# IDEA-CCNL/Fengshenbang-LM

Measured on NVIDIA H100. Metric: tokens_per_sec, higher is better.
Workload: dtype bf16

## Files before the change

fengshen-lm_b200/csrc/attention_bwd.cu:

```cuda
#include "host_common.h"
#include "ptx.cuh"

namespace fsb {

int make_attn_tmap(CUtensorMap* tm, const void* base, int64_t row_stride, int64_t width, int64_t seq, int64_t batch,
                   int box_rows);

constexpr int AB_THREADS = 384;
constexpr int AB_BM = 128;
constexpr int AB_BN = 64;
constexpr int AB_NDIAG = AB_BM + AB_BN - 1;
constexpr int AB_DSTRIDE = 192;

struct AttBwdParams {
  const float* lse;
  const float* delta;
  const uint8_t* kv_mask;
  const float* rel_bias;
  float* dbias_part;
  __nv_bfloat16 *dq, *dk, *dv;
  int64_t dq_row_stride, dk_row_stride, dv_row_stride, dq_head_stride, dk_head_stride, dv_head_stride;
  int q_head_stride, k_head_stride, v_head_stride, do_head_stride;
  int seq_q, seq_kv, nheads, batch, causal;
  float scale, scale_log2;
};

template <int D>
__global__ void __launch_bounds__(256) attn_delta_kernel(const __nv_bfloat16* __restrict__ o,
                                                         const __nv_bfloat16* __restrict__ dout, float* __restrict__ delta,
                                                         int64_t o_row_stride, int64_t o_head_stride,
                                                         int64_t do_row_stride, int64_t do_head_stride, int batch, int seq,
                                                         int nheads) {
  constexpr int G = D / 8;
  const int64_t gid = (blockIdx.x * int64_t(blockDim.x) + threadIdx.x) / G;
  const int gl = threadIdx.x % G;
  const int64_t total = int64_t(batch) * seq * nheads;
  float s = 0.f;
  int64_t bs = 0; int h = 0;
  if (gid < total) {
    h = int(gid % nheads);
    bs = gid / nheads;
    float a[8], b[8];
    unpack8(*reinterpret_cast<const uint4*>(o + bs * o_row_stride + h * o_head_stride + gl * 8), a);
    unpack8(*reinterpret_cast<const uint4*>(dout + bs * do_row_stride + h * do_head_stride + gl * 8), b);
#pragma unroll
    for (int j = 0; j < 8; ++j) s += a[j] * b[j];
  }
#pragma unroll
  for (int off = G / 2; off > 0; off >>= 1) s += __shfl_xor_sync(0xffffffffu, s, off);
  if (gid < total && gl == 0) {
    const int64_t b = bs / seq, sq = bs % seq;
    delta[(b * nheads + h) * seq + sq] = s;
  }
}

template <int D, bool kDS>
struct AttBwdSmem {
  static constexpr int BIG_BYTES = AB_BM * D * 2;
  static constexpr int SML_BYTES = AB_BN * D * 2;
  static constexpr int STAGES = 3;
  static constexpr int OFF_BIG0 = 0;
  static constexpr int OFF_BIG1 = OFF_BIG0 + BIG_BYTES;
  static constexpr int OFF_SML0 = OFF_BIG1 + BIG_BYTES;
  static constexpr int OFF_SML1 = OFF_SML0 + STAGES * SML_BYTES;
  static constexpr int OFF_DS = OFF_SML1 + STAGES * SML_BYTES;
  static constexpr int OFF_BAR = OFF_DS + (kDS ? (AB_BM * (AB_BN + 1) * 4 + 15) / 16 * 16 : 0);
  static constexpr int NBAR = 1 + 2 * STAGES;
  static constexpr int TOTAL = OFF_BAR + NBAR * 8 + 1024;
  static_assert(TOTAL <= 232448, "exceeds the 227 KB of shared memory a block can opt into on sm_90");
};

template <int D>
__device__ __forceinline__ void wgmma_rs_acc(float (&o)[D / 2], const uint32_t (&a)[4], uint64_t db) {
  if constexpr (D == 128) wgmma_rs_n128<1>(o, a, db, 1u);
  else wgmma_rs_n64<1>(o, a, db, 1u);
}
__device__ __forceinline__ uint32_t kslice(int kk, int rows) { return (kk / 4) * (rows * 128) + (kk % 4) * 32; }
__device__ __forceinline__ void to_frag(const float (&x)[32], int kk, uint32_t (&a)[4]) {
#pragma unroll
  for (int r = 0; r < 4; ++r) {
    const int i = 2 * kk + (r >> 1), h = r & 1;
    a[r] = pack_bf16x2(x[4 * i + 2 * h], x[4 * i + 2 * h + 1]);
  }
}

template <int D, bool kBias>
__global__ void __launch_bounds__(AB_THREADS, 1)
attn_bwd_dq_kernel(const __grid_constant__ CUtensorMap tmQ, const __grid_constant__ CUtensorMap tmdO,
                   const __grid_constant__ CUtensorMap tmK, const __grid_constant__ CUtensorMap tmV,
                   const AttBwdParams p) {
  using S = AttBwdSmem<D, kBias>;
  constexpr int STAGES = S::STAGES;
  extern __shared__ uint8_t smem_raw[];
  uint8_t* smem = reinterpret_cast<uint8_t*>((reinterpret_cast<uintptr_t>(smem_raw) + 1023) & ~uintptr_t(1023));
  uint64_t* bars = reinterpret_cast<uint64_t*>(smem + S::OFF_BAR);
  uint64_t* big_full = bars;
  uint64_t* sml_full = big_full + 1;
  uint64_t* sml_empty = sml_full + STAGES;

  const int warp = threadIdx.x >> 5, lane = threadIdx.x & 31;
  const int tile = gridDim.x - 1 - blockIdx.x;
  const int head = blockIdx.y, b = blockIdx.z;
  const int q0 = tile * AB_BM;
  const int n_all = (p.seq_kv + AB_BN - 1) / AB_BN;
  const int n_steps = p.causal ? min(n_all, (min(q0 + AB_BM, p.seq_q) + AB_BN - 1) / AB_BN) : n_all;

  if (threadIdx.x == 0) {
    tma_prefetch_desc(&tmQ); tma_prefetch_desc(&tmdO); tma_prefetch_desc(&tmK); tma_prefetch_desc(&tmV);
    mbar_init(big_full, 1);
    for (int i = 0; i < STAGES; ++i) { mbar_init(&sml_full[i], 1); mbar_init(&sml_empty[i], 8); }
    fence_barrier_init();
  }
  __syncthreads();

  if (warp < 4) {
    reg_dec<24>();
    if (threadIdx.x == 0) {
      const int qc = head * p.q_head_stride, dc = head * p.do_head_stride;
      const int kc = head * p.k_head_stride, vc = head * p.v_head_stride;
      mbar_expect_tx(big_full, 2 * S::BIG_BYTES);
#pragma unroll
      for (int h = 0; h < D / 64; ++h) {
        tma_load_3d(smem + S::OFF_BIG0 + h * (AB_BM * 128), &tmQ, big_full, qc + h * 64, q0, b);
        tma_load_3d(smem + S::OFF_BIG1 + h * (AB_BM * 128), &tmdO, big_full, dc + h * 64, q0, b);
      }
      int st = 0; uint32_t ph = 0;
      for (int j = 0; j < n_steps; ++j) {
        mbar_wait(&sml_empty[st], ph ^ 1);
        mbar_expect_tx(&sml_full[st], 2 * S::SML_BYTES);
#pragma unroll
        for (int h = 0; h < D / 64; ++h) {
          tma_load_3d(smem + S::OFF_SML0 + st * S::SML_BYTES + h * (AB_BN * 128), &tmK, &sml_full[st], kc + h * 64, j * AB_BN, b);
          tma_load_3d(smem + S::OFF_SML1 + st * S::SML_BYTES + h * (AB_BN * 128), &tmV, &sml_full[st], vc + h * 64, j * AB_BN, b);
        }
        if (++st == STAGES) { st = 0; ph ^= 1; }
      }
    }
    return;
  }

  reg_inc<240>();
  const int wg = (threadIdx.x >> 7) - 1;
  const int r_lo = wg * 64 + (warp & 3) * 16 + (lane >> 2);
  const int cq = 2 * (lane & 3);
  const uint64_t dsc_q = make_smem_desc_sw128(smem_u32(smem + S::OFF_BIG0) + wg * (64 * 128), 0, 1024);
  const uint64_t dsc_do = make_smem_desc_sw128(smem_u32(smem + S::OFF_BIG1) + wg * (64 * 128), 0, 1024);
  const uint64_t dsc_k = make_smem_desc_sw128(smem_u32(smem + S::OFF_SML0), 0, 1024);
  const uint64_t dsc_v = make_smem_desc_sw128(smem_u32(smem + S::OFF_SML1), 0, 1024);
  const uint64_t dsc_kmn = make_smem_desc_sw128(smem_u32(smem + S::OFF_SML0), AB_BN * 128, 1024);
  const uint8_t* mrow = p.kv_mask ? p.kv_mask + int64_t(b) * p.seq_kv : nullptr;
  const int n_rel = p.seq_q + p.seq_kv - 1;
  int q_row[2], kmax[2];
  float lse[2], delta[2];
  const float* brow[2];
#pragma unroll
  for (int h = 0; h < 2; ++h) {
    q_row[h] = q0 + r_lo + 8 * h;
    const bool ok = q_row[h] < p.seq_q;
    const int64_t si = (int64_t(b) * p.nheads + head) * p.seq_q + q_row[h];
    lse[h] = ok ? p.lse[si] : INFINITY;
    delta[h] = ok ? p.delta[si] : 0.f;
    kmax[h] = p.causal ? min(q_row[h], p.seq_kv - 1) : p.seq_kv - 1;
    brow[h] = kBias ? p.rel_bias + int64_t(head) * n_rel + (p.seq_q - 1 - min(q_row[h], p.seq_q - 1)) : nullptr;
  }
  float* dpart = kBias && p.dbias_part ? p.dbias_part + ((int64_t(b) * p.nheads + head) * gridDim.x + tile) * n_all * AB_DSTRIDE
                                       : nullptr;
  float dq[D / 2];
#pragma unroll
  for (int i = 0; i < D / 2; ++i) dq[i] = 0.f;

  mbar_wait(big_full, 0);
  for (int j = 0; j < n_steps; ++j) {
    const int st = j % STAGES;
    const uint32_t ph = (j / STAGES) & 1;
    const uint64_t sto = uint64_t(st) * (S::SML_BYTES >> 4);
    float s[32], dp[32];
    mbar_wait(&sml_full[st], ph);
    wgmma_fence();
#pragma unroll
    for (int kk = 0; kk < D / 16; ++kk)
      wgmma_ss_n64<0, 0>(s, dsc_q + (kslice(kk, AB_BM) >> 4), dsc_k + sto + (kslice(kk, AB_BN) >> 4), kk != 0 ? 1u : 0u);
#pragma unroll
    for (int kk = 0; kk < D / 16; ++kk)
      wgmma_ss_n64<0, 0>(dp, dsc_do + (kslice(kk, AB_BM) >> 4), dsc_v + sto + (kslice(kk, AB_BN) >> 4), kk != 0 ? 1u : 0u);
    wgmma_commit();
    wgmma_wait<0>();
    wgmma_fence_acc(s);
    wgmma_fence_acc(dp);
    const int c0 = j * AB_BN;
    const bool need_mask = (p.causal && c0 + AB_BN - 1 > q0 + wg * 64) || (c0 + AB_BN > p.seq_kv) || mrow;
#pragma unroll
    for (int i = 0; i < 8; ++i) {
#pragma unroll
      for (int e = 0; e < 4; ++e) {
        const int h = e >> 1, col = c0 + 8 * i + cq + (e & 1);
        float x = s[4 * i + e] * p.scale_log2 - lse[h];
        if constexpr (kBias) x = fmaf(__ldg(brow[h] + min(col, p.seq_kv - 1)), 1.4426950408889634f, x);
        float pe = ex2_approx(x);
        if (need_mask) {
          bool keep = col <= kmax[h];
          if (mrow != nullptr && keep) keep = mrow[col] != 0;
          pe = keep ? pe : 0.f;
        }
        s[4 * i + e] = pe * (dp[4 * i + e] - delta[h]);
      }
    }
    if constexpr (kBias) {
      if (dpart != nullptr) {
        float* tds = reinterpret_cast<float*>(smem + S::OFF_DS);
#pragma unroll
        for (int i = 0; i < 8; ++i)
#pragma unroll
          for (int e = 0; e < 4; ++e) tds[(r_lo + 8 * (e >> 1)) * (AB_BN + 1) + 8 * i + cq + (e & 1)] = s[4 * i + e];
        bar_sync(1, 256);
        const int t = threadIdx.x - 128;
        if (t < AB_NDIAG) {
          const int o = t - (AB_BM - 1);
          float acc = 0.f;
          for (int r = max(0, -o); r < min(AB_BM, AB_BN - o); ++r) acc += tds[r * (AB_BN + 2) + o];
          dpart[int64_t(j) * AB_DSTRIDE + t] = acc;
        }
        bar_sync(1, 256);
      }
    }
    uint32_t a[AB_BN / 16][4];
#pragma unroll
    for (int kk = 0; kk < AB_BN / 16; ++kk) to_frag(s, kk, a[kk]);
    wgmma_fence();
#pragma unroll
    for (int kk = 0; kk < AB_BN / 16; ++kk) wgmma_rs_acc<D>(dq, a[kk], dsc_kmn + sto + ((kk * 2048) >> 4));
    wgmma_commit();
    wgmma_wait<0>();
    wgmma_fence_acc(dq);
    __syncwarp();
    if (lane == 0) mbar_arrive(&sml_empty[st]);
  }
#pragma unroll
  for (int h = 0; h < 2; ++h) {
    if (q_row[h] >= p.seq_q) continue;
    __nv_bfloat16* dqp = p.dq + (int64_t(b) * p.seq_q + q_row[h]) * p.dq_row_stride + int64_t(head) * p.dq_head_stride + cq;
#pragma unroll
    for (int i = 0; i < D / 8; ++i)
      *reinterpret_cast<uint32_t*>(dqp + 8 * i) = pack_bf16x2(dq[4 * i + 2 * h] * p.scale, dq[4 * i + 2 * h + 1] * p.scale);
  }
}

template <int D, bool kBias>
__global__ void __launch_bounds__(AB_THREADS, 1)
attn_bwd_dkv_kernel(const __grid_constant__ CUtensorMap tmK, const __grid_constant__ CUtensorMap tmV,
                    const __grid_constant__ CUtensorMap tmQ, const __grid_constant__ CUtensorMap tmdO,
                    const AttBwdParams p) {
  using S = AttBwdSmem<D, false>;
  constexpr int STAGES = S::STAGES;
  extern __shared__ uint8_t smem_raw[];
  uint8_t* smem = reinterpret_cast<uint8_t*>((reinterpret_cast<uintptr_t>(smem_raw) + 1023) & ~uintptr_t(1023));
  uint64_t* bars = reinterpret_cast<uint64_t*>(smem + S::OFF_BAR);
  uint64_t* big_full = bars;
  uint64_t* sml_full = big_full + 1;
  uint64_t* sml_empty = sml_full + STAGES;

  const int warp = threadIdx.x >> 5, lane = threadIdx.x & 31;
  const int tile = blockIdx.x;
  const int head = blockIdx.y, b = blockIdx.z;
  const int kv0 = tile * AB_BM;
  const int n_q = (p.seq_q + AB_BN - 1) / AB_BN;
  const int i_start = p.causal ? min(n_q, kv0 / AB_BN) : 0;
  const int n_steps = n_q - i_start;

  if (threadIdx.x == 0) {
    tma_prefetch_desc(&tmQ); tma_prefetch_desc(&tmdO); tma_prefetch_desc(&tmK); tma_prefetch_desc(&tmV);
    mbar_init(big_full, 1);
    for (int i = 0; i < STAGES; ++i) { mbar_init(&sml_full[i], 1); mbar_init(&sml_empty[i], 8); }
    fence_barrier_init();
  }
  __syncthreads();

  if (warp < 4) {
    reg_dec<24>();
    if (threadIdx.x == 0) {
      const int qc = head * p.q_head_stride, dc = head * p.do_head_stride;
      const int kc = head * p.k_head_stride, vc = head * p.v_head_stride;
      mbar_expect_tx(big_full, 2 * S::BIG_BYTES);
#pragma unroll
      for (int h = 0; h < D / 64; ++h) {
        tma_load_3d(smem + S::OFF_BIG0 + h * (AB_BM * 128), &tmK, big_full, kc + h * 64, kv0, b);
        tma_load_3d(smem + S::OFF_BIG1 + h * (AB_BM * 128), &tmV, big_full, vc + h * 64, kv0, b);
      }
      int st = 0; uint32_t ph = 0;
      for (int i = 0; i < n_steps; ++i) {
        mbar_wait(&sml_empty[st], ph ^ 1);
        mbar_expect_tx(&sml_full[st], 2 * S::SML_BYTES);
#pragma unroll
        for (int h = 0; h < D / 64; ++h) {
          tma_load_3d(smem + S::OFF_SML0 + st * S::SML_BYTES + h * (AB_BN * 128), &tmQ, &sml_full[st], qc + h * 64,
                      (i_start + i) * AB_BN, b);
          tma_load_3d(smem + S::OFF_SML1 + st * S::SML_BYTES + h * (AB_BN * 128), &tmdO, &sml_full[st], dc + h * 64,
                      (i_start + i) * AB_BN, b);
        }
        if (++st == STAGES) { st = 0; ph ^= 1; }
      }
    }
    return;
  }

  reg_inc<240>();
  const int wg = (threadIdx.x >> 7) - 1;
  const int r_lo = wg * 64 + (warp & 3) * 16 + (lane >> 2);
  const int cq = 2 * (lane & 3);
  const uint64_t dsc_k = make_smem_desc_sw128(smem_u32(smem + S::OFF_BIG0) + wg * (64 * 128), 0, 1024);
  const uint64_t dsc_v = make_smem_desc_sw128(smem_u32(smem + S::OFF_BIG1) + wg * (64 * 128), 0, 1024);
  const uint64_t dsc_q = make_smem_desc_sw128(smem_u32(smem + S::OFF_SML0), 0, 1024);
  const uint64_t dsc_do = make_smem_desc_sw128(smem_u32(smem + S::OFF_SML1), 0, 1024);
  const uint64_t dsc_qmn = make_smem_desc_sw128(smem_u32(smem + S::OFF_SML0), AB_BN * 128, 1024);
  const uint64_t dsc_domn = make_smem_desc_sw128(smem_u32(smem + S::OFF_SML1), AB_BN * 128, 1024);
  const int64_t stat_base = (int64_t(b) * p.nheads + head) * p.seq_q;
  const int n_rel = p.seq_q + p.seq_kv - 1;
  int kv_row[2];
  bool row_ok[2];
  const float* bkey[2];
#pragma unroll
  for (int h = 0; h < 2; ++h) {
    kv_row[h] = kv0 + r_lo + 8 * h;
    row_ok[h] = kv_row[h] < p.seq_kv && (p.kv_mask == nullptr || p.kv_mask[int64_t(b) * p.seq_kv + kv_row[h]] != 0);
    bkey[h] = kBias ? p.rel_bias + int64_t(head) * n_rel + (min(kv_row[h], p.seq_kv - 1) + p.seq_q - 1) : nullptr;
  }
  float dv[D / 2], dk[D / 2];
#pragma unroll
  for (int i = 0; i < D / 2; ++i) { dv[i] = 0.f; dk[i] = 0.f; }

  mbar_wait(big_full, 0);
  for (int i = 0; i < n_steps; ++i) {
    const int st = i % STAGES;
    const uint32_t ph = (i / STAGES) & 1;
    const uint64_t sto = uint64_t(st) * (S::SML_BYTES >> 4);
    const int qt0 = (i_start + i) * AB_BN;
    float s[32], dp[32];
    mbar_wait(&sml_full[st], ph);
    wgmma_fence();
#pragma unroll
    for (int kk = 0; kk < D / 16; ++kk)
      wgmma_ss_n64<0, 0>(s, dsc_k + (kslice(kk, AB_BM) >> 4), dsc_q + sto + (kslice(kk, AB_BN) >> 4), kk != 0 ? 1u : 0u);
#pragma unroll
    for (int kk = 0; kk < D / 16; ++kk)
      wgmma_ss_n64<0, 0>(dp, dsc_v + (kslice(kk, AB_BM) >> 4), dsc_do + sto + (kslice(kk, AB_BN) >> 4), kk != 0 ? 1u : 0u);
    wgmma_commit();
    wgmma_wait<0>();
    wgmma_fence_acc(s);
    wgmma_fence_acc(dp);
    const bool need_causal = p.causal && (qt0 < kv0 + AB_BM - 1);
#pragma unroll
    for (int ii = 0; ii < 8; ++ii) {
#pragma unroll
      for (int c = 0; c < 2; ++c) {
        const int qi = qt0 + 8 * ii + cq + c;
        const bool q_ok = qi < p.seq_q;
        const float lse_c = q_ok ? __ldg(p.lse + stat_base + qi) : INFINITY;
        const float del_c = q_ok ? __ldg(p.delta + stat_base + qi) : 0.f;
#pragma unroll
        for (int h = 0; h < 2; ++h) {
          const int e = 2 * h + c;
          float arg = s[4 * ii + e] * p.scale_log2 - lse_c;
          if constexpr (kBias) arg = fmaf(__ldg(bkey[h] - min(qi, p.seq_q - 1)), 1.4426950408889634f, arg);
          float x = ex2_approx(arg);
          const bool keep = row_ok[h] && !(need_causal && qi < kv_row[h]);
          x = keep ? x : 0.f;
          s[4 * ii + e] = x;
          dp[4 * ii + e] = x * (dp[4 * ii + e] - del_c);
        }
      }
    }
    uint32_t pa[AB_BN / 16][4], da[AB_BN / 16][4];
#pragma unroll
    for (int kk = 0; kk < AB_BN / 16; ++kk) { to_frag(s, kk, pa[kk]); to_frag(dp, kk, da[kk]); }
    wgmma_fence();
#pragma unroll
    for (int kk = 0; kk < AB_BN / 16; ++kk) wgmma_rs_acc<D>(dv, pa[kk], dsc_domn + sto + ((kk * 2048) >> 4));
#pragma unroll
    for (int kk = 0; kk < AB_BN / 16; ++kk) wgmma_rs_acc<D>(dk, da[kk], dsc_qmn + sto + ((kk * 2048) >> 4));
    wgmma_commit();
    wgmma_wait<0>();
    wgmma_fence_acc(dv);
    wgmma_fence_acc(dk);
    __syncwarp();
    if (lane == 0) mbar_arrive(&sml_empty[st]);
  }
#pragma unroll
  for (int h = 0; h < 2; ++h) {
    if (kv_row[h] >= p.seq_kv) continue;
    __nv_bfloat16* dvp = p.dv + (int64_t(b) * p.seq_kv + kv_row[h]) * p.dv_row_stride + int64_t(head) * p.dv_head_stride + cq;
    __nv_bfloat16* dkp = p.dk + (int64_t(b) * p.seq_kv + kv_row[h]) * p.dk_row_stride + int64_t(head) * p.dk_head_stride + cq;
#pragma unroll
    for (int i = 0; i < D / 8; ++i) {
      *reinterpret_cast<uint32_t*>(dvp + 8 * i) = pack_bf16x2(dv[4 * i + 2 * h], dv[4 * i + 2 * h + 1]);
      *reinterpret_cast<uint32_t*>(dkp + 8 * i) = pack_bf16x2(dk[4 * i + 2 * h] * p.scale, dk[4 * i + 2 * h + 1] * p.scale);
    }
  }
}

__global__ void __launch_bounds__(128) attn_dbias_reduce_kernel(const float* __restrict__ part, float* __restrict__ part2,
                                                                int batch, int nheads, int seq_q, int seq_kv, int causal,
                                                                int n_qtiles, int bsplit) {
  const int n_rel = seq_q + seq_kv - 1;
  const int i = blockIdx.x * blockDim.x + threadIdx.x;
  const int h = blockIdx.y, sp = blockIdx.z;
  if (i >= n_rel) return;
  const int d = i - (seq_q - 1);
  const int n_all = (seq_kv + AB_BN - 1) / AB_BN;
  const int b0 = int(int64_t(batch) * sp / bsplit), b1 = int(int64_t(batch) * (sp + 1) / bsplit);
  float acc = 0.f;
  for (int b = b0; b < b1; ++b) {
    for (int tile = 0; tile < n_qtiles; ++tile) {
      const int q0 = tile * AB_BM;
      const int n_steps = causal ? min(n_all, (min(q0 + AB_BM, seq_q) + AB_BN - 1) / AB_BN) : n_all;
      const float* base = part + ((int64_t(b) * nheads + h) * n_qtiles + tile) * n_all * AB_DSTRIDE;
      const int hi = d + q0 + (AB_BM - 1), lo = d + q0 - (AB_BN - 1);
      if (hi < 0) continue;
      const int j_lo = lo <= 0 ? 0 : (lo + AB_BN - 1) / AB_BN, j_hi = min(n_steps - 1, hi / AB_BN);
      for (int j = j_lo; j <= j_hi; ++j) acc += base[int64_t(j) * AB_DSTRIDE + (hi - j * AB_BN)];
    }
  }
  part2[(int64_t(sp) * nheads + h) * n_rel + i] = acc;
}
__global__ void __launch_bounds__(128) attn_dbias_final_kernel(const float* __restrict__ part2, float* __restrict__ dbias,
                                                               int nheads, int n_rel, int bsplit) {
  const int i = blockIdx.x * blockDim.x + threadIdx.x;
  const int h = blockIdx.y;
  if (i >= n_rel) return;
  float acc = dbias[int64_t(h) * n_rel + i];
  for (int sp = 0; sp < bsplit; ++sp) acc += part2[(int64_t(sp) * nheads + h) * n_rel + i];
  dbias[int64_t(h) * n_rel + i] = acc;
}
static inline int dbias_bsplit(int batch) { return batch < 16 ? batch : 16; }
static inline size_t dbias_part_floats(int64_t batch, int64_t seq_q, int64_t seq_kv, int nheads) {
  const int64_t n_qt = (seq_q + AB_BM - 1) / AB_BM, n_all = (seq_kv + AB_BN - 1) / AB_BN;
  return size_t(batch) * nheads * n_qt * n_all * AB_DSTRIDE;
}

template <int D, bool kBias>
static int launch_attn_bwd(const void* q, const void* k, const void* v, const void* o, const void* dout,
                           int64_t q_rs, int64_t k_rs, int64_t v_rs, int64_t o_rs, int64_t do_rs, int64_t o_hs,
                           float* delta, AttBwdParams& p, float* drel_bias, float* part2, cudaStream_t st) {
  using SQ = AttBwdSmem<D, kBias>;
  using SK = AttBwdSmem<D, false>;
  static bool configured = false;
  if (!configured) {
    cudaError_t e1 = cudaFuncSetAttribute(attn_bwd_dq_kernel<D, kBias>, cudaFuncAttributeMaxDynamicSharedMemorySize, SQ::TOTAL);
    cudaError_t e2 = cudaFuncSetAttribute(attn_bwd_dkv_kernel<D, kBias>, cudaFuncAttributeMaxDynamicSharedMemorySize, SK::TOTAL);
    if (e1 != cudaSuccess || e2 != cudaSuccess) {
      set_error("sdpa_bwd: cudaFuncSetAttribute(%d / %d) failed", SQ::TOTAL, SK::TOTAL);
      return FSB_ERR_CUDA;
    }
    configured = true;
  }
  {
    const int64_t groups = int64_t(p.batch) * p.seq_q * p.nheads;
    const int64_t threads = groups * (D / 8);
    attn_delta_kernel<D><<<unsigned((threads + 255) / 256), 256, 0, st>>>(
        (const __nv_bfloat16*)o, (const __nv_bfloat16*)dout, delta, o_rs, o_hs, do_rs, p.do_head_stride, p.batch, p.seq_q,
        p.nheads);
    FSB_CUDA_LAUNCH_CHECK();
  }
  CUtensorMap tq128, tdo128, tk64, tv64, tk128, tv128, tq64, tdo64;
  int rc;
  const int64_t wq = int64_t(p.nheads - 1) * p.q_head_stride + D, wk = int64_t(p.nheads - 1) * p.k_head_stride + D;
  const int64_t wv = int64_t(p.nheads - 1) * p.v_head_stride + D, wdo = int64_t(p.nheads - 1) * p.do_head_stride + D;
  if ((rc = make_attn_tmap(&tq128, q, q_rs, wq, p.seq_q, p.batch, AB_BM))) return rc;
  if ((rc = make_attn_tmap(&tdo128, dout, do_rs, wdo, p.seq_q, p.batch, AB_BM))) return rc;
  if ((rc = make_attn_tmap(&tk64, k, k_rs, wk, p.seq_kv, p.batch, AB_BN))) return rc;
  if ((rc = make_attn_tmap(&tv64, v, v_rs, wv, p.seq_kv, p.batch, AB_BN))) return rc;
  if ((rc = make_attn_tmap(&tk128, k, k_rs, wk, p.seq_kv, p.batch, AB_BM))) return rc;
  if ((rc = make_attn_tmap(&tv128, v, v_rs, wv, p.seq_kv, p.batch, AB_BM))) return rc;
  if ((rc = make_attn_tmap(&tq64, q, q_rs, wq, p.seq_q, p.batch, AB_BN))) return rc;
  if ((rc = make_attn_tmap(&tdo64, dout, do_rs, wdo, p.seq_q, p.batch, AB_BN))) return rc;
  {
    dim3 grid((p.seq_q + AB_BM - 1) / AB_BM, p.nheads, p.batch);
    attn_bwd_dq_kernel<D, kBias><<<grid, AB_THREADS, SQ::TOTAL, st>>>(tq128, tdo128, tk64, tv64, p);
    FSB_CUDA_LAUNCH_CHECK();
    if (kBias && drel_bias != nullptr) {
      const int n_rel = p.seq_q + p.seq_kv - 1, bs = dbias_bsplit(p.batch);
      attn_dbias_reduce_kernel<<<dim3((n_rel + 127) / 128, p.nheads, bs), 128, 0, st>>>(
          p.dbias_part, part2, p.batch, p.nheads, p.seq_q, p.seq_kv, p.causal, int(grid.x), bs);
      FSB_CUDA_LAUNCH_CHECK();
      attn_dbias_final_kernel<<<dim3((n_rel + 127) / 128, p.nheads), 128, 0, st>>>(part2, drel_bias, p.nheads, n_rel, bs);
      FSB_CUDA_LAUNCH_CHECK();
    }
  }
  {
    dim3 grid((p.seq_kv + AB_BM - 1) / AB_BM, p.nheads, p.batch);
    attn_bwd_dkv_kernel<D, kBias><<<grid, AB_THREADS, SK::TOTAL, st>>>(tk128, tv128, tq64, tdo64, p);
    FSB_CUDA_LAUNCH_CHECK();
  }
  return FSB_OK;
}

}

using namespace fsb;

extern "C" int fsb_sdpa_bwd(const void* q, const void* k, const void* v, const void* o, const void* dout,
                            const float* lse, float* delta, void* dq, void* dk, void* dv, int64_t batch, int64_t seq_q,
                            int64_t seq_kv, int nheads, int head_dim, int64_t q_row_stride, int64_t k_row_stride,
                            int64_t v_row_stride, int64_t o_row_stride, int64_t do_row_stride, int64_t dq_row_stride,
                            int64_t dk_row_stride, int64_t dv_row_stride, int64_t q_head_stride, int64_t k_head_stride,
                            int64_t v_head_stride, int64_t o_head_stride, int64_t do_head_stride,
                            int64_t dq_head_stride, int64_t dk_head_stride, int64_t dv_head_stride, float scale,
                            int causal, const uint8_t* kv_mask, const float* rel_bias, float* drel_bias, void* workspace,
                            size_t workspace_bytes, fsb_stream_t st) {
  FSB_REQUIRE(q && k && v && o && dout && lse && delta && dq && dk && dv, "sdpa_bwd: null pointer");
  FSB_REQUIRE(head_dim == 64 || head_dim == 128, "sdpa_bwd: head_dim %d unsupported (64 or 128)", head_dim);
  FSB_REQUIRE(batch > 0 && seq_q > 0 && seq_kv > 0 && nheads > 0 && batch < 65536 && nheads < 65536, "sdpa_bwd: bad dims");
  FSB_REQUIRE(!causal || seq_q == seq_kv, "sdpa_bwd: causal needs seq_q == seq_kv");
  FSB_REQUIRE(aligned16(q) && aligned16(k) && aligned16(v) && aligned16(o) && aligned16(dout) && aligned16(dq) &&
                  aligned16(dk) && aligned16(dv),
              "sdpa_bwd: 16-byte alignment required");
  FSB_REQUIRE((q_row_stride | k_row_stride | v_row_stride | o_row_stride | do_row_stride | dq_row_stride |
               dk_row_stride | dv_row_stride | q_head_stride | k_head_stride | v_head_stride | o_head_stride |
               do_head_stride | dq_head_stride | dk_head_stride | dv_head_stride) % 8 == 0,
              "sdpa_bwd: strides must be multiples of 8 elements");
  FSB_REQUIRE(drel_bias == nullptr || rel_bias != nullptr, "sdpa_bwd: drel_bias without rel_bias");
  AttBwdParams p;
  p.lse = lse; p.delta = delta; p.kv_mask = kv_mask;
  p.rel_bias = rel_bias; p.dbias_part = nullptr;
  float* part2 = nullptr;
  if (drel_bias != nullptr) {
    const size_t need = fsb_sdpa_bwd_workspace_bytes(batch, seq_q, seq_kv, nheads);
    FSB_REQUIRE(workspace != nullptr && workspace_bytes >= need && aligned16(workspace),
                "sdpa_bwd: the bias gradient needs a %zu-byte workspace (fsb_sdpa_bwd_workspace_bytes); got %zu", need,
                workspace_bytes);
    p.dbias_part = static_cast<float*>(workspace);
    part2 = p.dbias_part + dbias_part_floats(batch, seq_q, seq_kv, nheads);
  }
  p.dq = (__nv_bfloat16*)dq; p.dk = (__nv_bfloat16*)dk; p.dv = (__nv_bfloat16*)dv;
  p.dq_row_stride = dq_row_stride; p.dk_row_stride = dk_row_stride; p.dv_row_stride = dv_row_stride;
  p.dq_head_stride = dq_head_stride; p.dk_head_stride = dk_head_stride; p.dv_head_stride = dv_head_stride;
  p.q_head_stride = int(q_head_stride); p.k_head_stride = int(k_head_stride); p.v_head_stride = int(v_head_stride);
  p.do_head_stride = int(do_head_stride);
  p.seq_q = int(seq_q); p.seq_kv = int(seq_kv); p.nheads = nheads; p.batch = int(batch); p.causal = causal;
  p.scale = scale; p.scale_log2 = scale * 1.4426950408889634f;
#define FSB_BWD(DD, BB)                                                                                                  \
  launch_attn_bwd<DD, BB>(q, k, v, o, dout, q_row_stride, k_row_stride, v_row_stride, o_row_stride, do_row_stride,       \
                          o_head_stride, delta, p, drel_bias, part2, (cudaStream_t)st)
  if (rel_bias != nullptr) return head_dim == 128 ? FSB_BWD(128, true) : FSB_BWD(64, true);
  return head_dim == 128 ? FSB_BWD(128, false) : FSB_BWD(64, false);
#undef FSB_BWD
}

extern "C" size_t fsb_sdpa_bwd_workspace_bytes(int64_t batch, int64_t seq_q, int64_t seq_kv, int nheads) {
  if (batch <= 0 || seq_q <= 0 || seq_kv <= 0 || nheads <= 0) return 0;
  return (fsb::dbias_part_floats(batch, seq_q, seq_kv, nheads) +
          size_t(fsb::dbias_bsplit(int(batch))) * nheads * size_t(seq_q + seq_kv - 1)) * sizeof(float);
}
```

fengshen-lm_b200/csrc/attention_fwd.cu:

```cuda
#include <stdlib.h>

#include "host_common.h"
#include "ptx.cuh"

namespace fsb {

constexpr int ATT_BQ = 128;
constexpr int ATT_BKV = 128;
constexpr int ATT_THREADS = 384;

template <int D>
struct AttFwdSmem {
  static constexpr int STAGES = D == 128 ? 2 : 3;
  static constexpr int Q_BYTES = ATT_BQ * D * 2;
  static constexpr int KV_BYTES = ATT_BKV * D * 2;
  static constexpr int OFF_Q = 0;
  static constexpr int OFF_K = OFF_Q + Q_BYTES;
  static constexpr int OFF_V = OFF_K + STAGES * KV_BYTES;
  static constexpr int OFF_BAR = OFF_V + STAGES * KV_BYTES;
  static constexpr int NBAR = 1 + 3 * STAGES;
  static constexpr int TOTAL = OFF_BAR + NBAR * 8 + 1024;
  static_assert(TOTAL <= 232448, "exceeds the 227 KB of shared memory a block can opt into on sm_90");
};

struct AttFwdParams {
  __nv_bfloat16* o;
  float* lse;
  const uint8_t* kv_mask;
  const float* rel_bias;
  int64_t o_row_stride, o_head_stride;
  int q_head_stride, k_head_stride, v_head_stride;
  int seq_q, seq_kv, nheads, batch;
  int causal;
  float scale_log2;
};

template <int D>
__device__ __forceinline__ void wgmma_rs_d(float (&o)[D / 2], const uint32_t (&a)[4], uint64_t db) {
  if constexpr (D == 128) wgmma_rs_n128<1>(o, a, db, 1u);
  else wgmma_rs_n64<1>(o, a, db, 1u);
}

template <int D, bool kBias>
__global__ void __launch_bounds__(ATT_THREADS, 1)
attn_fwd_kernel(const __grid_constant__ CUtensorMap tmQ, const __grid_constant__ CUtensorMap tmK,
                const __grid_constant__ CUtensorMap tmV, const AttFwdParams p) {
  using S = AttFwdSmem<D>;
  constexpr int STAGES = S::STAGES;

  extern __shared__ uint8_t smem_raw[];
  uint8_t* smem = reinterpret_cast<uint8_t*>((reinterpret_cast<uintptr_t>(smem_raw) + 1023) & ~uintptr_t(1023));
  uint64_t* bars = reinterpret_cast<uint64_t*>(smem + S::OFF_BAR);
  uint64_t* q_full = bars;
  uint64_t* k_full = q_full + 1;
  uint64_t* v_full = k_full + STAGES;
  uint64_t* kv_empty = v_full + STAGES;

  const int warp = threadIdx.x >> 5, lane = threadIdx.x & 31;
  const int tile = gridDim.x - 1 - blockIdx.x;
  const int head = blockIdx.y, b = blockIdx.z;
  const int q0 = tile * ATT_BQ;
  const int n_all = (p.seq_kv + ATT_BKV - 1) / ATT_BKV;
  const int n_kv = p.causal ? min(n_all, (min(q0 + ATT_BQ, p.seq_q) + ATT_BKV - 1) / ATT_BKV) : n_all;

  if (threadIdx.x == 0) {
    tma_prefetch_desc(&tmQ); tma_prefetch_desc(&tmK); tma_prefetch_desc(&tmV);
    mbar_init(q_full, 1);
    for (int i = 0; i < STAGES; ++i) {
      mbar_init(&k_full[i], 1); mbar_init(&v_full[i], 1);
      mbar_init(&kv_empty[i], 8);
    }
    fence_barrier_init();
  }
  __syncthreads();

  if (warp < 4) {
    reg_dec<24>();
    if (threadIdx.x == 0) {
      const int qc = head * p.q_head_stride, kc = head * p.k_head_stride, vc = head * p.v_head_stride;
      mbar_expect_tx(q_full, S::Q_BYTES);
#pragma unroll
      for (int h = 0; h < D / 64; ++h) tma_load_3d(smem + S::OFF_Q + h * (ATT_BQ * 128), &tmQ, q_full, qc + h * 64, q0, b);
      int st = 0; uint32_t ph = 0;
      for (int j = 0; j < n_kv; ++j) {
        mbar_wait(&kv_empty[st], ph ^ 1);
        mbar_expect_tx(&k_full[st], S::KV_BYTES);
#pragma unroll
        for (int h = 0; h < D / 64; ++h)
          tma_load_3d(smem + S::OFF_K + st * S::KV_BYTES + h * (ATT_BKV * 128), &tmK, &k_full[st], kc + h * 64, j * ATT_BKV, b);
        mbar_expect_tx(&v_full[st], S::KV_BYTES);
#pragma unroll
        for (int h = 0; h < D / 64; ++h)
          tma_load_3d(smem + S::OFF_V + st * S::KV_BYTES + h * (ATT_BKV * 128), &tmV, &v_full[st], vc + h * 64, j * ATT_BKV, b);
        if (++st == STAGES) { st = 0; ph ^= 1; }
      }
    }
    return;
  }

  reg_inc<240>();
  const int wg = (threadIdx.x >> 7) - 1;
  const int r_lo = wg * 64 + (warp & 3) * 16 + (lane >> 2);
  const int cq = 2 * (lane & 3);
  const uint64_t dsc_q = make_smem_desc_sw128(smem_u32(smem + S::OFF_Q) + wg * (64 * 128), 0, 1024);
  const uint64_t dsc_k = make_smem_desc_sw128(smem_u32(smem + S::OFF_K), 0, 1024);
  const uint64_t dsc_v = make_smem_desc_sw128(smem_u32(smem + S::OFF_V), ATT_BKV * 128, 1024);
  const uint8_t* mrow = p.kv_mask ? p.kv_mask + int64_t(b) * p.seq_kv : nullptr;
  const float sc = p.scale_log2;
  const int n_rel = p.seq_q + p.seq_kv - 1;
  int q_row[2], kmax[2];
  const float* brow[2];
#pragma unroll
  for (int h = 0; h < 2; ++h) {
    q_row[h] = q0 + r_lo + 8 * h;
    kmax[h] = p.causal ? min(q_row[h], p.seq_kv - 1) : p.seq_kv - 1;
    brow[h] = kBias ? p.rel_bias + int64_t(head) * n_rel + (p.seq_q - 1 - min(q_row[h], p.seq_q - 1)) : nullptr;
  }
  float o[D / 2];
#pragma unroll
  for (int i = 0; i < D / 2; ++i) o[i] = 0.f;
  float m[2] = {-INFINITY, -INFINITY}, l[2] = {0.f, 0.f};

  mbar_wait(q_full, 0);
  for (int j = 0; j < n_kv; ++j) {
    const int st = j % STAGES;
    const uint32_t ph = (j / STAGES) & 1;
    float s[ATT_BKV / 2];
    mbar_wait(&k_full[st], ph);
    wgmma_fence();
#pragma unroll
    for (int kk = 0; kk < D / 16; ++kk)
      wgmma_ss_n128<0, 0>(s, dsc_q + (((kk / 4) * (ATT_BQ * 128) + (kk % 4) * 32) >> 4),
                          dsc_k + ((st * S::KV_BYTES + (kk / 4) * (ATT_BKV * 128) + (kk % 4) * 32) >> 4), kk != 0 ? 1u : 0u);
    wgmma_commit();
    wgmma_wait<0>();
    wgmma_fence_acc(s);

    const int c0 = j * ATT_BKV;
    const bool need_mask = (p.causal && c0 + ATT_BKV - 1 > q0 + wg * 64) || (c0 + ATT_BKV > p.seq_kv) || mrow;
#pragma unroll
    for (int i = 0; i < ATT_BKV / 8; ++i) {
#pragma unroll
      for (int e = 0; e < 4; ++e) {
        const int h = e >> 1, col = c0 + 8 * i + cq + (e & 1);
        float x;
        if constexpr (kBias) x = fmaf(__ldg(brow[h] + min(col, p.seq_kv - 1)), 1.4426950408889634f, s[4 * i + e] * sc);
        else x = s[4 * i + e] * sc;
        if (need_mask) {
          bool keep = col <= kmax[h];
          if (mrow != nullptr && keep) keep = mrow[col] != 0;
          x = keep ? x : -INFINITY;
        }
        s[4 * i + e] = x;
      }
    }
    float neg_m[2];
#pragma unroll
    for (int h = 0; h < 2; ++h) {
      float mx = -INFINITY;
#pragma unroll
      for (int i = 0; i < ATT_BKV / 8; ++i) mx = fmaxf(mx, fmaxf(s[4 * i + 2 * h], s[4 * i + 2 * h + 1]));
      mx = fmaxf(mx, __shfl_xor_sync(0xffffffffu, mx, 1));
      mx = fmaxf(mx, __shfl_xor_sync(0xffffffffu, mx, 2));
      const float m_new = fmaxf(m[h], mx);
      const float f = (m_new == -INFINITY) ? 1.f : ex2_approx(m[h] - m_new);
      l[h] *= f;
#pragma unroll
      for (int i = 0; i < D / 8; ++i) { o[4 * i + 2 * h] *= f; o[4 * i + 2 * h + 1] *= f; }
      m[h] = m_new;
      neg_m[h] = (m_new == -INFINITY) ? 0.f : -m_new;
    }
    uint32_t pa[ATT_BKV / 16][4];
#pragma unroll
    for (int kk = 0; kk < ATT_BKV / 16; ++kk) {
#pragma unroll
      for (int r = 0; r < 4; ++r) {
        const int h = r & 1, i = 2 * kk + (r >> 1);
        const float a = ex2_approx(s[4 * i + 2 * h] + neg_m[h]), c = ex2_approx(s[4 * i + 2 * h + 1] + neg_m[h]);
        l[h] += a + c;
        pa[kk][r] = pack_bf16x2(a, c);
      }
    }
    mbar_wait(&v_full[st], ph);
    wgmma_fence();
#pragma unroll
    for (int kk = 0; kk < ATT_BKV / 16; ++kk)
      wgmma_rs_d<D>(o, pa[kk], dsc_v + ((st * S::KV_BYTES + kk * 2048) >> 4));
    wgmma_commit();
    wgmma_wait<0>();
    wgmma_fence_acc(o);
    __syncwarp();
    if (lane == 0) mbar_arrive(&kv_empty[st]);
  }

#pragma unroll
  for (int h = 0; h < 2; ++h) {
    float lr = l[h];
    lr += __shfl_xor_sync(0xffffffffu, lr, 1);
    lr += __shfl_xor_sync(0xffffffffu, lr, 2);
    if (q_row[h] >= p.seq_q) continue;
    const float inv = lr > 0.f ? 1.f / lr : 0.f;
    __nv_bfloat16* op = p.o + (int64_t(b) * p.seq_q + q_row[h]) * p.o_row_stride + int64_t(head) * p.o_head_stride + cq;
#pragma unroll
    for (int i = 0; i < D / 8; ++i)
      *reinterpret_cast<uint32_t*>(op + 8 * i) = pack_bf16x2(o[4 * i + 2 * h] * inv, o[4 * i + 2 * h + 1] * inv);
    if ((lane & 3) == 0)
      p.lse[(int64_t(b) * p.nheads + head) * p.seq_q + q_row[h]] = lr > 0.f ? m[h] + log2f(lr) : INFINITY;
  }
}

int make_attn_tmap(CUtensorMap* tm, const void* base, int64_t row_stride, int64_t width, int64_t seq, int64_t batch,
                   int box_rows) {
  uint64_t dims[3] = {uint64_t(width), uint64_t(seq), uint64_t(batch)};
  uint64_t strides[2] = {uint64_t(row_stride) * 2, uint64_t(seq) * uint64_t(row_stride) * 2};
  uint32_t box[3] = {64, uint32_t(box_rows), 1};
  return make_tmap_bf16(tm, base, 3, dims, strides, box);
}

template <int D, bool kBias>
static int launch_attn_fwd(const CUtensorMap& tq, const CUtensorMap& tk, const CUtensorMap& tv, const AttFwdParams& p,
                           cudaStream_t st) {
  using S = AttFwdSmem<D>;
  static bool configured = false;
  auto kern = attn_fwd_kernel<D, kBias>;
  if (!configured) {
    cudaError_t e = cudaFuncSetAttribute(kern, cudaFuncAttributeMaxDynamicSharedMemorySize, S::TOTAL);
    if (e != cudaSuccess) {
      set_error("sdpa_fwd: cudaFuncSetAttribute(%d) failed: %s", S::TOTAL, cudaGetErrorString(e));
      return FSB_ERR_CUDA;
    }
    configured = true;
  }
  dim3 grid((p.seq_q + ATT_BQ - 1) / ATT_BQ, p.nheads, p.batch);
  kern<<<grid, ATT_THREADS, S::TOTAL, st>>>(tq, tk, tv, p);
  FSB_CUDA_LAUNCH_CHECK();
  return FSB_OK;
}

}

using namespace fsb;

extern "C" int fsb_sdpa_fwd(const void* q, const void* k, const void* v, void* o, float* lse, int64_t batch,
                            int64_t seq_q, int64_t seq_kv, int nheads, int head_dim, int64_t q_row_stride,
                            int64_t k_row_stride, int64_t v_row_stride, int64_t o_row_stride, int64_t q_head_stride,
                            int64_t k_head_stride, int64_t v_head_stride, int64_t o_head_stride, float scale, int causal,
                            const uint8_t* kv_mask, const float* rel_bias, fsb_stream_t st) {
  FSB_REQUIRE(q && k && v && o && lse, "sdpa_fwd: null pointer");
  FSB_REQUIRE(head_dim == 64 || head_dim == 128, "sdpa_fwd: head_dim %d unsupported (64 or 128)", head_dim);
  FSB_REQUIRE(batch > 0 && seq_q > 0 && seq_kv > 0 && nheads > 0 && batch < 65536 && nheads < 65536, "sdpa_fwd: bad dims");
  FSB_REQUIRE(!causal || seq_q == seq_kv, "sdpa_fwd: causal needs seq_q == seq_kv");
  FSB_REQUIRE(scale > 0.f, "sdpa_fwd: softmax scale must be positive");
  FSB_REQUIRE(aligned16(q) && aligned16(k) && aligned16(v) && aligned16(o), "sdpa_fwd: 16-byte alignment required");
  FSB_REQUIRE((q_row_stride | k_row_stride | v_row_stride | o_row_stride | q_head_stride | k_head_stride |
               v_head_stride | o_head_stride) % 8 == 0,
              "sdpa_fwd: strides must be multiples of 8 elements");
  CUtensorMap tq, tk, tv;
  int rc;
  if ((rc = make_attn_tmap(&tq, q, q_row_stride, (nheads - 1) * q_head_stride + head_dim, seq_q, batch, ATT_BQ))) return rc;
  if ((rc = make_attn_tmap(&tk, k, k_row_stride, (nheads - 1) * k_head_stride + head_dim, seq_kv, batch, ATT_BKV))) return rc;
  if ((rc = make_attn_tmap(&tv, v, v_row_stride, (nheads - 1) * v_head_stride + head_dim, seq_kv, batch, ATT_BKV))) return rc;
  AttFwdParams p;
  p.o = (__nv_bfloat16*)o; p.lse = lse; p.kv_mask = kv_mask; p.rel_bias = rel_bias;
  p.o_row_stride = o_row_stride; p.o_head_stride = o_head_stride;
  p.q_head_stride = int(q_head_stride); p.k_head_stride = int(k_head_stride); p.v_head_stride = int(v_head_stride);
  p.seq_q = int(seq_q); p.seq_kv = int(seq_kv); p.nheads = nheads; p.batch = int(batch);
  p.causal = causal;
  p.scale_log2 = scale * 1.4426950408889634f;
  if (rel_bias != nullptr)
    return head_dim == 128 ? launch_attn_fwd<128, true>(tq, tk, tv, p, (cudaStream_t)st)
                           : launch_attn_fwd<64, true>(tq, tk, tv, p, (cudaStream_t)st);
  return head_dim == 128 ? launch_attn_fwd<128, false>(tq, tk, tv, p, (cudaStream_t)st)
                         : launch_attn_fwd<64, false>(tq, tk, tv, p, (cudaStream_t)st);
}
```

Measured before the change: 447,600.

## Software-pipeline attention backward WGMMAs and stage LSE/delta in shared memory

The dq and dkv backward kernels now issue the next tile's S/dP wgmma before the previous tile's dQ (or dK/dV) wgmma. This lets softmax-gradient math overlap tensor-core work, replacing the full wait between the two GEMM phases. In the dkv kernel a producer warp loads LSE and delta per q-tile into a new shared-memory stage, and the full barrier now expects the extra arrivals, so consumers skip per-element global loads. Masking in forward and backward is split into unmasked, causal-only and key-mask variants to remove branches in the hot loop. The change adds register pressure and barrier complexity, and pipelining is enabled only for some template configurations.

Result: faster. 465,000, median of 6 (+3.9%).

```diff
diff --git a/fengshen-lm_b200/csrc/attention_bwd.cu b/fengshen-lm_b200/csrc/attention_bwd.cu
--- a/fengshen-lm_b200/csrc/attention_bwd.cu
+++ b/fengshen-lm_b200/csrc/attention_bwd.cu
@@ -63,7 +63,8 @@
   static constexpr int OFF_BIG1 = OFF_BIG0 + BIG_BYTES;
   static constexpr int OFF_SML0 = OFF_BIG1 + BIG_BYTES;
   static constexpr int OFF_SML1 = OFF_SML0 + STAGES * SML_BYTES;
-  static constexpr int OFF_DS = OFF_SML1 + STAGES * SML_BYTES;
+  static constexpr int OFF_STAT = OFF_SML1 + STAGES * SML_BYTES;
+  static constexpr int OFF_DS = OFF_STAT + STAGES * 2 * AB_BN * 4;
   static constexpr int OFF_BAR = OFF_DS + (kDS ? (AB_BM * (AB_BN + 1) * 4 + 15) / 16 * 16 : 0);
   static constexpr int NBAR = 1 + 2 * STAGES;
   static constexpr int TOTAL = OFF_BAR + NBAR * 8 + 1024;
@@ -169,13 +170,12 @@
 #pragma unroll
   for (int i = 0; i < D / 2; ++i) dq[i] = 0.f;
 
-  mbar_wait(big_full, 0);
-  for (int j = 0; j < n_steps; ++j) {
+  float s[32], dp[32];
+  uint32_t a[AB_BN / 16][4];
+  auto issue_sdp = [&](int j) {
     const int st = j % STAGES;
-    const uint32_t ph = (j / STAGES) & 1;
     const uint64_t sto = uint64_t(st) * (S::SML_BYTES >> 4);
-    float s[32], dp[32];
-    mbar_wait(&sml_full[st], ph);
+    mbar_wait(&sml_full[st], (j / STAGES) & 1);
     wgmma_fence();
 #pragma unroll
     for (int kk = 0; kk < D / 16; ++kk)
@@ -184,26 +184,47 @@
     for (int kk = 0; kk < D / 16; ++kk)
       wgmma_ss_n64<0, 0>(dp, dsc_do + (kslice(kk, AB_BM) >> 4), dsc_v + sto + (kslice(kk, AB_BN) >> 4), kk != 0 ? 1u : 0u);
     wgmma_commit();
-    wgmma_wait<0>();
-    wgmma_fence_acc(s);
-    wgmma_fence_acc(dp);
+  };
+  auto issue_dq = [&](int j) {
+    const uint64_t sto = uint64_t(j % STAGES) * (S::SML_BYTES >> 4);
+    wgmma_fence();
+#pragma unroll
+    for (int kk = 0; kk < AB_BN / 16; ++kk) wgmma_rs_acc<D>(dq, a[kk], dsc_kmn + sto + ((kk * 2048) >> 4));
+    wgmma_commit();
+  };
+  auto form_ds = [&](int j) {
     const int c0 = j * AB_BN;
     const bool need_mask = (p.causal && c0 + AB_BN - 1 > q0 + wg * 64) || (c0 + AB_BN > p.seq_kv) || mrow;
-#pragma unroll
-    for (int i = 0; i < 8; ++i) {
-#pragma unroll
-      for (int e = 0; e < 4; ++e) {
-        const int h = e >> 1, col = c0 + 8 * i + cq + (e & 1);
-        float x = s[4 * i + e] * p.scale_log2 - lse[h];
-        if constexpr (kBias) x = fmaf(__ldg(brow[h] + min(col, p.seq_kv - 1)), 1.4426950408889634f, x);
-        float pe = ex2_approx(x);
-        if (need_mask) {
-          bool keep = col <= kmax[h];
-          if (mrow != nullptr && keep) keep = mrow[col] != 0;
-          pe = keep ? pe : 0.f;
+    auto prob = [&](int i, int e) {
+      const int h = e >> 1, col = c0 + 8 * i + cq + (e & 1);
+      float x = s[4 * i + e] * p.scale_log2 - lse[h];
+      if constexpr (kBias) x = fmaf(__ldg(brow[h] + min(col, p.seq_kv - 1)), 1.4426950408889634f, x);
+      return ex2_approx(x);
+    };
+    if (!need_mask) {
+#pragma unroll
+      for (int i = 0; i < 8; ++i)
+#pragma unroll
+        for (int e = 0; e < 4; ++e) s[4 * i + e] = prob(i, e) * (dp[4 * i + e] - delta[e >> 1]);
+    } else if (mrow == nullptr) {
+#pragma unroll
+      for (int i = 0; i < 8; ++i)
+#pragma unroll
+        for (int e = 0; e < 4; ++e) {
+          const int col = c0 + 8 * i + cq + (e & 1);
+          const float pe = prob(i, e);
+          s[4 * i + e] = (col <= kmax[e >> 1] ? pe : 0.f) * (dp[4 * i + e] - delta[e >> 1]);
         }
-        s[4 * i + e] = pe * (dp[4 * i + e] - delta[h]);
-      }
+    } else {
+#pragma unroll
+      for (int i = 0; i < 8; ++i)
+#pragma unroll
+        for (int e = 0; e < 4; ++e) {
+          const int col = c0 + 8 * i + cq + (e & 1);
+          const float pe = prob(i, e);
+          const bool keep = (col <= kmax[e >> 1]) & (mrow[min(col, p.seq_kv - 1)] != 0);
+          s[4 * i + e] = (keep ? pe : 0.f) * (dp[4 * i + e] - delta[e >> 1]);
+        }
     }
     if constexpr (kBias) {
       if (dpart != nullptr) {
@@ -223,17 +244,52 @@
         bar_sync(1, 256);
       }
     }
-    uint32_t a[AB_BN / 16][4];
+  };
+  auto release = [&](int j) {
+    __syncwarp();
+    if (lane == 0) mbar_arrive(&sml_empty[j % STAGES]);
+  };
+
+  mbar_wait(big_full, 0);
+  if constexpr (!kBias) {
+    issue_sdp(0);
+    wgmma_wait<0>();
+    wgmma_fence_acc(s);
+    wgmma_fence_acc(dp);
+    form_ds(0);
 #pragma unroll
     for (int kk = 0; kk < AB_BN / 16; ++kk) to_frag(s, kk, a[kk]);
-    wgmma_fence();
-#pragma unroll
-    for (int kk = 0; kk < AB_BN / 16; ++kk) wgmma_rs_acc<D>(dq, a[kk], dsc_kmn + sto + ((kk * 2048) >> 4));
-    wgmma_commit();
+    for (int j = 1; j < n_steps; ++j) {
+      issue_sdp(j);
+      issue_dq(j - 1);
+      wgmma_wait<1>();
+      wgmma_fence_acc(s);
+      wgmma_fence_acc(dp);
+      form_ds(j);
+      wgmma_wait<0>();
+      wgmma_fence_acc(dq);
+      release(j - 1);
+#pragma unroll
+      for (int kk = 0; kk < AB_BN / 16; ++kk) to_frag(s, kk, a[kk]);
+    }
+    issue_dq(n_steps - 1);
     wgmma_wait<0>();
     wgmma_fence_acc(dq);
-    __syncwarp();
-    if (lane == 0) mbar_arrive(&sml_empty[st]);
+    release(n_steps - 1);
+  } else {
+    for (int j = 0; j < n_steps; ++j) {
+      issue_sdp(j);
+      wgmma_wait<0>();
+      wgmma_fence_acc(s);
+      wgmma_fence_acc(dp);
+      form_ds(j);
+#pragma unroll
+      for (int kk = 0; kk < AB_BN / 16; ++kk) to_frag(s, kk, a[kk]);
+      issue_dq(j);
+      wgmma_wait<0>();
+      wgmma_fence_acc(dq);
+      release(j);
+    }
   }
 #pragma unroll
   for (int h = 0; h < 2; ++h) {
@@ -270,13 +326,30 @@
   if (threadIdx.x == 0) {
     tma_prefetch_desc(&tmQ); tma_prefetch_desc(&tmdO); tma_prefetch_desc(&tmK); tma_prefetch_desc(&tmV);
     mbar_init(big_full, 1);
-    for (int i = 0; i < STAGES; ++i) { mbar_init(&sml_full[i], 1); mbar_init(&sml_empty[i], 8); }
+    for (int i = 0; i < STAGES; ++i) { mbar_init(&sml_full[i], 1 + 32); mbar_init(&sml_empty[i], 8); }
     fence_barrier_init();
   }
   __syncthreads();
 
   if (warp < 4) {
     reg_dec<24>();
+    if (warp == 1) {
+      const int64_t stat_base = (int64_t(b) * p.nheads + head) * p.seq_q;
+      float* stat = reinterpret_cast<float*>(smem + S::OFF_STAT);
+      int st = 0; uint32_t ph = 0;
+      for (int i = 0; i < n_steps; ++i) {
+        mbar_wait(&sml_empty[st], ph ^ 1);
+#pragma unroll
+        for (int c = 0; c < 2; ++c) {
+          const int qc = c * 32 + lane, qi = (i_start + i) * AB_BN + qc;
+          const bool q_ok = qi < p.seq_q;
+          stat[st * 2 * AB_BN + qc] = q_ok ? __ldg(p.lse + stat_base + qi) : INFINITY;
+          stat[st * 2 * AB_BN + AB_BN + qc] = q_ok ? __ldg(p.delta + stat_base + qi) : 0.f;
+        }
+        mbar_arrive(&sml_full[st]);
+        if (++st == STAGES) { st = 0; ph ^= 1; }
+      }
+    }
     if (threadIdx.x == 0) {
       const int qc = head * p.q_head_stride, dc = head * p.do_head_stride;
       const int kc = head * p.k_head_stride, vc = head * p.v_head_stride;
@@ -313,7 +386,6 @@
   const uint64_t dsc_do = make_smem_desc_sw128(smem_u32(smem + S::OFF_SML1), 0, 1024);
   const uint64_t dsc_qmn = make_smem_desc_sw128(smem_u32(smem + S::OFF_SML0), AB_BN * 128, 1024);
   const uint64_t dsc_domn = make_smem_desc_sw128(smem_u32(smem + S::OFF_SML1), AB_BN * 128, 1024);
-  const int64_t stat_base = (int64_t(b) * p.nheads + head) * p.seq_q;
   const int n_rel = p.seq_q + p.seq_kv - 1;
   int kv_row[2];
   bool row_ok[2];
@@ -328,14 +400,13 @@
 #pragma unroll
   for (int i = 0; i < D / 2; ++i) { dv[i] = 0.f; dk[i] = 0.f; }
 
-  mbar_wait(big_full, 0);
-  for (int i = 0; i < n_steps; ++i) {
+  float s[32], dp[32];
+  uint32_t pa[AB_BN / 16][4], da[AB_BN / 16][4];
+  const float* stat = reinterpret_cast<const float*>(smem + S::OFF_STAT);
+  auto issue_sdp = [&](int i) {
     const int st = i % STAGES;
-    const uint32_t ph = (i / STAGES) & 1;
     const uint64_t sto = uint64_t(st) * (S::SML_BYTES >> 4);
-    const int qt0 = (i_start + i) * AB_BN;
-    float s[32], dp[32];
-    mbar_wait(&sml_full[st], ph);
+    mbar_wait(&sml_full[st], (i / STAGES) & 1);
     wgmma_fence();
 #pragma unroll
     for (int kk = 0; kk < D / 16; ++kk)
@@ -344,18 +415,27 @@
     for (int kk = 0; kk < D / 16; ++kk)
       wgmma_ss_n64<0, 0>(dp, dsc_v + (kslice(kk, AB_BM) >> 4), dsc_do + sto + (kslice(kk, AB_BN) >> 4), kk != 0 ? 1u : 0u);
     wgmma_commit();
-    wgmma_wait<0>();
-    wgmma_fence_acc(s);
-    wgmma_fence_acc(dp);
+  };
+  auto issue_dkv = [&](int i) {
+    const uint64_t sto = uint64_t(i % STAGES) * (S::SML_BYTES >> 4);
+    wgmma_fence();
+#pragma unroll
+    for (int kk = 0; kk < AB_BN / 16; ++kk) wgmma_rs_acc<D>(dv, pa[kk], dsc_domn + sto + ((kk * 2048) >> 4));
+#pragma unroll
+    for (int kk = 0; kk < AB_BN / 16; ++kk) wgmma_rs_acc<D>(dk, da[kk], dsc_qmn + sto + ((kk * 2048) >> 4));
+    wgmma_commit();
+  };
+  auto form_p_ds = [&](int i) {
+    const int qt0 = (i_start + i) * AB_BN;
+    const float* st_lse = stat + (i % STAGES) * 2 * AB_BN;
     const bool need_causal = p.causal && (qt0 < kv0 + AB_BM - 1);
 #pragma unroll
     for (int ii = 0; ii < 8; ++ii) {
 #pragma unroll
       for (int c = 0; c < 2; ++c) {
         const int qi = qt0 + 8 * ii + cq + c;
-        const bool q_ok = qi < p.seq_q;
-        const float lse_c = q_ok ? __ldg(p.lse + stat_base + qi) : INFINITY;
-        const float del_c = q_ok ? __ldg(p.delta + stat_base + qi) : 0.f;
+        const float lse_c = st_lse[8 * ii + cq + c];
+        const float del_c = st_lse[AB_BN + 8 * ii + cq + c];
 #pragma unroll
         for (int h = 0; h < 2; ++h) {
           const int e = 2 * h + c;
@@ -369,20 +449,56 @@
         }
       }
     }
-    uint32_t pa[AB_BN / 16][4], da[AB_BN / 16][4];
+  };
+  auto pack = [&]() {
 #pragma unroll
     for (int kk = 0; kk < AB_BN / 16; ++kk) { to_frag(s, kk, pa[kk]); to_frag(dp, kk, da[kk]); }
-    wgmma_fence();
-#pragma unroll
-    for (int kk = 0; kk < AB_BN / 16; ++kk) wgmma_rs_acc<D>(dv, pa[kk], dsc_domn + sto + ((kk * 2048) >> 4));
-#pragma unroll
-    for (int kk = 0; kk < AB_BN / 16; ++kk) wgmma_rs_acc<D>(dk, da[kk], dsc_qmn + sto + ((kk * 2048) >> 4));
-    wgmma_commit();
+  };
+  auto release = [&](int i) {
+    __syncwarp();
+    if (lane == 0) mbar_arrive(&sml_empty[i % STAGES]);
+  };
+
+  mbar_wait(big_full, 0);
+  if constexpr (D == 64 && !kBias) {
+    issue_sdp(0);
+    wgmma_wait<0>();
+    wgmma_fence_acc(s);
+    wgmma_fence_acc(dp);
+    form_p_ds(0);
+    pack();
+    for (int i = 1; i < n_steps; ++i) {
+      issue_sdp(i);
+      issue_dkv(i - 1);
+      wgmma_wait<1>();
+      wgmma_fence_acc(s);
+      wgmma_fence_acc(dp);
+      form_p_ds(i);
+      wgmma_wait<0>();
+      wgmma_fence_acc(dv);
+      wgmma_fence_acc(dk);
+      release(i - 1);
+      pack();
+    }
+    issue_dkv(n_steps - 1);
     wgmma_wait<0>();
     wgmma_fence_acc(dv);
     wgmma_fence_acc(dk);
-    __syncwarp();
-    if (lane == 0) mbar_arrive(&sml_empty[st]);
+    release(n_steps - 1);
+  } else {
+    for (int i = 0; i < n_steps; ++i) {
+      issue_sdp(i);
+      wgmma_wait<0>();
+      wgmma_fence_acc(s);
+      wgmma_fence_acc(dp);
+      form_p_ds(i);
+      pack();
+      issue_dkv(i);
+      wgmma_wait<0>();
+      wgmma_fence_acc(dv);
+      wgmma_fence_acc(dk);
+      release(i);
+    }
   }
 #pragma unroll
   for (int h = 0; h < 2; ++h) {
diff --git a/fengshen-lm_b200/csrc/attention_fwd.cu b/fengshen-lm_b200/csrc/attention_fwd.cu
--- a/fengshen-lm_b200/csrc/attention_fwd.cu
+++ b/fengshen-lm_b200/csrc/attention_fwd.cu
@@ -138,21 +138,49 @@
 
     const int c0 = j * ATT_BKV;
     const bool need_mask = (p.causal && c0 + ATT_BKV - 1 > q0 + wg * 64) || (c0 + ATT_BKV > p.seq_kv) || mrow;
-#pragma unroll
-    for (int i = 0; i < ATT_BKV / 8; ++i) {
-#pragma unroll
-      for (int e = 0; e < 4; ++e) {
-        const int h = e >> 1, col = c0 + 8 * i + cq + (e & 1);
-        float x;
-        if constexpr (kBias) x = fmaf(__ldg(brow[h] + min(col, p.seq_kv - 1)), 1.4426950408889634f, s[4 * i + e] * sc);
-        else x = s[4 * i + e] * sc;
-        if (need_mask) {
-          bool keep = col <= kmax[h];
-          if (mrow != nullptr && keep) keep = mrow[col] != 0;
-          x = keep ? x : -INFINITY;
+    auto scaled = [&](int i, int e) {
+      const int h = e >> 1, col = c0 + 8 * i + cq + (e & 1);
+      if constexpr (kBias) return fmaf(__ldg(brow[h] + min(col, p.seq_kv - 1)), 1.4426950408889634f, s[4 * i + e] * sc);
+      else return s[4 * i + e] * sc;
+    };
+    if constexpr (kBias && D == 128) {
+#pragma unroll
+      for (int i = 0; i < ATT_BKV / 8; ++i)
+#pragma unroll
+        for (int e = 0; e < 4; ++e) {
+          const int col = c0 + 8 * i + cq + (e & 1);
+          float x = scaled(i, e);
+          if (need_mask) {
+            bool keep = col <= kmax[e >> 1];
+            if (mrow != nullptr && keep) keep = mrow[col] != 0;
+            x = keep ? x : -INFINITY;
+          }
+          s[4 * i + e] = x;
         }
-        s[4 * i + e] = x;
-      }
+    } else if (!need_mask) {
+#pragma unroll
+      for (int i = 0; i < ATT_BKV / 8; ++i)
+#pragma unroll
+        for (int e = 0; e < 4; ++e) s[4 * i + e] = scaled(i, e);
+    } else if (mrow == nullptr) {
+#pragma unroll
+      for (int i = 0; i < ATT_BKV / 8; ++i)
+#pragma unroll
+        for (int e = 0; e < 4; ++e) {
+          const int col = c0 + 8 * i + cq + (e & 1);
+          const float x = scaled(i, e);
+          s[4 * i + e] = col <= kmax[e >> 1] ? x : -INFINITY;
+        }
+    } else {
+#pragma unroll
+      for (int i = 0; i < ATT_BKV / 8; ++i)
+#pragma unroll
+        for (int e = 0; e < 4; ++e) {
+          const int col = c0 + 8 * i + cq + (e & 1);
+          const float x = scaled(i, e);
+          const bool keep = (col <= kmax[e >> 1]) & (mrow[min(col, p.seq_kv - 1)] != 0);
+          s[4 * i + e] = keep ? x : -INFINITY;
+        }
     }
     float neg_m[2];
 #pragma unroll
```
